# saithepaithewhyyy/Stochastic-Gradient-MCMC-for-non-linear-state-models---MTH422

Measured on AMD Instinct MI355X. Metric: SGLD steps/sec (T=1000, N=1000 particles), higher is better.
Workload: dtype f64

## Files before the change

### stochastic-gradient-mcmc-for-non-linear-state-models---mth422_amd/csrc/pfg_models.hpp

```cpp
#pragma once
#include "pfg_math.hpp"

namespace pfg {

template <int MODEL> struct ModelDims;
template <> struct ModelDims<PFG_MODEL_SVM>   { static constexpr int NS = 1, H = 3; };
template <> struct ModelDims<PFG_MODEL_GARCH> { static constexpr int NS = 2, H = 4; };
template <> struct ModelDims<PFG_MODEL_LGSSM> { static constexpr int NS = 1, H = 4; };

template <typename REAL> struct Consts {
    REAL LRinv, iLRinv, Rinv, R, logLRinv, c0;
    REAL A, C, LQinv, iLQinv, Qinv;
    REAL opt_sd, opt_prec, opt_var, opt_logvar;
    REAL mu, phi, lam, alpha, beta, gamma;
    REAL logalpha, logLQinv;
};

template <int MODEL, typename REAL>
__device__ __forceinline__ Consts<REAL> make_consts(const double *__restrict__ th) {
    Consts<double> d = {};
    d.c0 = -0.5 * LOG_2PI;
    double LRinv;
    if (MODEL == PFG_MODEL_SVM) {
        d.A = th[0]; d.LQinv = th[1]; LRinv = th[2];
    } else if (MODEL == PFG_MODEL_LGSSM) {
        d.A = th[0]; d.C = th[1]; d.LQinv = th[2]; LRinv = th[3];
    } else {
        LRinv = th[3];
        d.mu = exp(th[0]);
        d.phi = 1.0 / (1.0 + exp(-th[1]));
        d.lam = 1.0 / (1.0 + exp(-th[2]));
        d.alpha = d.mu * (1.0 - d.phi);
        d.beta = d.phi * d.lam;
        d.gamma = d.phi * (1.0 - d.lam);
    }
    d.LRinv = LRinv;
    d.iLRinv = 1.0 / LRinv;
    d.Rinv = LRinv * LRinv + 1e-16;
    d.R = 1.0 / d.Rinv;
    d.logLRinv = log(LRinv);
    if (MODEL != PFG_MODEL_GARCH) {
        d.iLQinv = 1.0 / d.LQinv;
        d.Qinv = d.LQinv * d.LQinv + 1e-16;
        d.logLQinv = log(d.LQinv);
    } else {
        d.logalpha = log(d.alpha);
    }
    if (MODEL == PFG_MODEL_LGSSM) {
        d.opt_prec = d.Qinv + (d.C * d.C) * d.Rinv;
        d.opt_sd = pow(d.opt_prec, -0.5);
        d.opt_var = 1.0 / d.Qinv + 1.0 / d.Rinv;
        d.opt_logvar = log(d.opt_var);
    }
    {
        double *f = reinterpret_cast<double *>(&d);
#pragma unroll
        for (int q = 0; q < (int)(sizeof(d) / sizeof(double)); ++q) f[q] = uniform_f64(f[q]);
    }
    Consts<REAL> c;
    c.LRinv = (REAL)d.LRinv; c.iLRinv = (REAL)d.iLRinv; c.Rinv = (REAL)d.Rinv; c.R = (REAL)d.R;
    c.logLRinv = (REAL)d.logLRinv; c.c0 = (REAL)d.c0;
    c.A = (REAL)d.A; c.C = (REAL)d.C; c.LQinv = (REAL)d.LQinv; c.iLQinv = (REAL)d.iLQinv;
    c.Qinv = (REAL)d.Qinv;
    c.opt_sd = (REAL)d.opt_sd; c.opt_prec = (REAL)d.opt_prec; c.opt_var = (REAL)d.opt_var;
    c.opt_logvar = (REAL)d.opt_logvar;
    c.mu = (REAL)d.mu; c.phi = (REAL)d.phi; c.lam = (REAL)d.lam;
    c.alpha = (REAL)d.alpha; c.beta = (REAL)d.beta; c.gamma = (REAL)d.gamma;
    c.logalpha = (REAL)d.logalpha; c.logLQinv = (REAL)d.logLQinv;
    return c;
}

template <int MODEL, int KERNEL, int STAT, typename REAL, typename MATH>
__device__ __forceinline__ void particle_step(const Consts<REAL> &c, const MATH &mth, const REAL *xp,
                                              REAL y, REAL z, REAL *xn, REAL &lw, REAL *add) {
    constexpr int H = ModelDims<MODEL>::H;
    const REAL half = (REAL)0.5;
#pragma unroll
    for (int h = 0; h < H; ++h) add[h] = (REAL)0;
    if (MODEL == PFG_MODEL_SVM) {
        REAL xpA = xp[0] * c.A;
        REAL x1 = c.iLQinv * z + xpA;
        REAL e = mth.exp_finite(-x1);
        REAL y2 = y * y;
#ifdef PFG_FAST_ALGEBRA
        const REAL k0 = c.c0 + c.logLRinv, ke = (-half * y2) * c.Rinv;
        lw = fma(ke, e, fma(-half, x1, k0));
#else
        lw = ((c.c0 + ((-half * y2) * e) * c.Rinv) + c.logLRinv) + (-half * x1);
#endif
        xn[0] = x1;
        if (STAT == PFG_STAT_SCORE) {
            REAL dx = x1 - c.A * xp[0];
            add[2] = (c.Qinv * dx) * xp[0];
            add[1] = c.iLQinv - (dx * dx) * c.LQinv;
#ifdef PFG_FAST_ALGEBRA
            add[0] = fma(-(y2 * c.LRinv), e, c.iLRinv);
#else
            REAL dy2 = y2 * e;
            add[0] = c.iLRinv - dy2 * c.LRinv;
#endif
        } else {
            add[0] = x1; add[1] = x1 * x1; add[2] = xp[0] * x1;
        }
    } else if (MODEL == PFG_MODEL_LGSSM) {
        REAL x1;
        if (KERNEL == PFG_KERNEL_PRIOR) {
            x1 = c.iLQinv * z + xp[0] * c.A;
            REAL diff = y - c.C * x1;
            lw = (c.c0 + (-half * (diff * diff)) * c.Rinv) + c.logLRinv;
        } else {
#ifdef PFG_FAST_ALGEBRA
            const REAL rprec = (REAL)1 / c.opt_prec, rvar = (REAL)1 / c.opt_var;
            REAL mp = (xp[0] * c.A) * c.Qinv + (y * c.C) * c.Rinv;
            x1 = fma(c.opt_sd, z, mp * rprec);
            REAL diff = y - c.A * xp[0];
            lw = fma(-half * (diff * diff), rvar, -half * (REAL)LOG_2PI - half * c.opt_logvar);
#else
            REAL mp = (xp[0] * c.A) * c.Qinv + (y * c.C) * c.Rinv;
            x1 = c.opt_sd * z + mp / c.opt_prec;
            REAL diff = y - c.A * xp[0];
            lw = ((-half * (diff * diff)) / c.opt_var - half * (REAL)LOG_2PI) - half * c.opt_logvar;
#endif
        }
        xn[0] = x1;
        if (STAT == PFG_STAT_SCORE) {
            REAL dx = x1 - c.A * xp[0];
            add[3] = (c.Qinv * dx) * xp[0];
            add[1] = c.iLQinv - (dx * dx) * c.LQinv;
            REAL dy = y - c.C * x1;
            add[2] = (c.Rinv * dy) * x1;
            add[0] = c.iLRinv - (dy * dy) * c.LRinv;
        } else {
            add[0] = x1; add[1] = x1 * x1; add[2] = xp[0] * x1;
        }
    } else {
        REAL xx = xp[0] * xp[0];
        REAL s2 = (c.alpha + c.beta * xx) + c.gamma * xp[1];
        REAL x1;
        if (KERNEL == PFG_KERNEL_PRIOR) {
#ifdef PFG_FAST_ALGEBRA
            x1 = mth.sqrt_pos(s2) * z;
#else
            x1 = mth.sqrt(s2) * z;
#endif
            REAL diff = y - x1;
            lw = (c.c0 + (-half * (diff * diff)) * c.Rinv) + c.logLRinv;
        } else {
#ifdef PFG_FAST_ALGEBRA
            const REAL v2 = s2 + c.R;
            const REAL rv2 = mth.rcp_pos(v2);
            const REAL var = (s2 * c.R) * rv2;
            x1 = fma(mth.sqrt_pos(var), z, var * (y * c.Rinv));
            lw = fma(-half * (y * y), rv2, c.c0) + (-half * mth.log(v2));
#else
            REAL var = (REAL)1 / (c.Rinv + (REAL)1 / s2);
            REAL mean = var * (y * c.Rinv);
            x1 = mean + mth.sqrt(var) * z;
            REAL v2 = s2 + c.R;
            lw = (c.c0 + (-half * (y * y)) / v2) + (-half * mth.log(v2));
#endif
        }
        xn[0] = x1; xn[1] = s2;
        if (STAT == PFG_STAT_SCORE) {
            REAL v = s2;
#ifdef PFG_FAST_ALGEBRA
            const REAL rv = mth.rcp_pos(v);
            const REAL gv = (-half * (v - x1 * x1)) * (rv * rv);
            const REAL omp = (REAL)1 - c.phi, oml_ = (REAL)1 - c.lam;
            add[1] = gv * (omp * c.mu);
            add[2] = (gv * fma(c.lam, xx, fma(oml_, xp[1], -c.mu))) * (omp * c.phi);
            add[3] = (gv * (xx - xp[1])) * ((c.phi * oml_) * c.lam);
            REAL dy = y - x1;
            add[0] = fma(-(dy * dy), c.LRinv, c.iLRinv);
#else
            REAL gv = (-half * (v - x1 * x1)) / (v * v);
            add[1] = (gv * ((REAL)1 - c.phi)) * c.mu;
            add[2] = ((gv * ((-c.mu + c.lam * xx) + ((REAL)1 - c.lam) * xp[1])) * ((REAL)1 - c.phi)) * c.phi;
            add[3] = (((gv * c.phi) * (xx - xp[1])) * ((REAL)1 - c.lam)) * c.lam;
            REAL dy = y - x1;
            add[0] = c.iLRinv - (dy * dy) * c.LRinv;
#endif
        } else {
            REAL x2 = x1 * x1;
            add[0] = x1; add[1] = x2; add[2] = x2 * x2;
        }
    }
}

template <int MODEL, int STAT, typename REAL>
__device__ __forceinline__ void additive_stat(const Consts<REAL> &c, const REAL *xp, const REAL *xn, REAL y,
                                              REAL aux, REAL *add) {
    constexpr int H = ModelDims<MODEL>::H;
    const REAL half = (REAL)0.5;
#pragma unroll
    for (int h = 0; h < H; ++h) add[h] = (REAL)0;
    if (STAT != PFG_STAT_SCORE) {
        if (MODEL == PFG_MODEL_GARCH) { REAL x2 = xn[0] * xn[0]; add[0] = xn[0]; add[1] = x2; add[2] = x2 * x2; }
        else { add[0] = xn[0]; add[1] = xn[0] * xn[0]; add[2] = xp[0] * xn[0]; }
        return;
    }
    if (MODEL == PFG_MODEL_SVM) {
        REAL dx = xn[0] - c.A * xp[0];
        add[2] = (c.Qinv * dx) * xp[0];
        add[1] = c.iLQinv - (dx * dx) * c.LQinv;
        add[0] = c.iLRinv - ((y * y) * aux) * c.LRinv;
    } else if (MODEL == PFG_MODEL_LGSSM) {
        REAL dx = xn[0] - c.A * xp[0];
        add[3] = (c.Qinv * dx) * xp[0];
        add[1] = c.iLQinv - (dx * dx) * c.LQinv;
        REAL dy = y - c.C * xn[0];
        add[2] = (c.Rinv * dy) * xn[0];
        add[0] = c.iLRinv - (dy * dy) * c.LRinv;
    } else {
        REAL xx = xp[0] * xp[0];
        REAL v = xn[1];
        REAL gv = (-half * (v - xn[0] * xn[0])) / (v * v);
        add[1] = (gv * ((REAL)1 - c.phi)) * c.mu;
        add[2] = ((gv * ((-c.mu + c.lam * xx) + ((REAL)1 - c.lam) * xp[1])) * ((REAL)1 - c.phi)) * c.phi;
        add[3] = (((gv * c.phi) * (xx - xp[1])) * ((REAL)1 - c.lam)) * c.lam;
        REAL dy = y - xn[0];
        add[0] = c.iLRinv - (dy * dy) * c.LRinv;
    }
}

template <int MODEL, typename REAL, typename MATH>
__device__ __forceinline__ REAL backward_log_ratio(const Consts<REAL> &c, const MATH &mth, const REAL *xp,
                                                   const REAL *xn) {
    const REAL half = (REAL)0.5;
    if (MODEL == PFG_MODEL_GARCH) {
        REAL s2 = (c.alpha + c.beta * (xp[0] * xp[0])) + c.gamma * xp[1];
        REAL ll = ((-half * (xn[0] * xn[0])) / s2 - half * (REAL)LOG_2PI) - half * mth.log(s2);
        return ll - (-half * (REAL)LOG_2PI - half * c.logalpha);
    }
    REAL diff = xn[0] - c.A * xp[0];
    REAL ll = ((-half * (diff * diff)) * c.Qinv + -half * (REAL)LOG_2PI) + c.logLQinv;
    return ll - (-half * (REAL)LOG_2PI + c.logLQinv);
}

}
```

### stochastic-gradient-mcmc-for-non-linear-state-models---mth422_amd/csrc/pfg_reg_kernel.hpp

```cpp
#pragma once
#include "pfg_models.hpp"

namespace pfg {

__host__ __device__ __forceinline__ constexpr int cdf_phys(int i) { return i + (i >> 5); }
__host__ __device__ constexpr bool fast_layout(int NT, bool PP) { return PP || NT <= 512 || NT == 1024; }

#ifndef PFG_OPT_PADSTATE
#define PFG_OPT_PADSTATE 1
#endif
template <typename REAL, int RNG> __host__ __device__ constexpr int state_pad() {
    return (PFG_OPT_PADSTATE && RNG == PFG_RNG_DEVICE) ? (int)(8 / sizeof(REAL)) : 0;
}

template <int NW> __device__ __forceinline__ void block_sync() {
    if (NW == 1) {
        __builtin_amdgcn_fence(__ATOMIC_RELEASE, "wavefront");
        __builtin_amdgcn_wave_barrier();
        __builtin_amdgcn_fence(__ATOMIC_ACQUIRE, "wavefront");
    } else {
        __syncthreads();
    }
}
template <int NT, int PPT> struct RegLayout {
    static constexpr int NW = NT / WAVE;
    static constexpr int RED = PPT * NW + NW + PFG_MAX_STAT * NW + 8;
};

template <int MODEL, typename REAL, int NT, int PPT, int RNG, bool PP, int MODE = 0>
__host__ __device__ inline size_t reg_kernel_lds_bytes(int N) {
    constexpr bool PARIS = (MODE == MODE_PARIS || MODE == MODE_N2);
    constexpr bool FAST = fast_layout(NT, PP);
    size_t NL = FAST ? (size_t)NT * PPT : (size_t)(N + WAVE - 1) / WAVE * WAVE;
    size_t NC = FAST ? (size_t)NT * PPT + (size_t)NT * PPT / 32 : NL;
    constexpr bool BLK = FAST && RNG == PFG_RNG_DEVICE && MODE == MODE_PLAIN && (PPT & (PPT - 1)) == 0;
    const size_t NLS = NL + (FAST ? state_pad<REAL, RNG>() : 0);
    return (NC * (BLK ? 4 : 8) + 15) / 16 * 16 + (PP ? 2 : 1) * NLS * (ModelDims<MODEL>::NS + ModelDims<MODEL>::H) * sizeof(REAL) +
           (size_t)RegLayout<NT, PPT>::RED * 8 + tab_bytes<REAL, RNG, FAST>() +
           (PARIS ? NL * 8 + NL * 4 + 3 * NL * 4 : 0);
}

#ifndef PFG_OCC64
#define PFG_OCC64 4
#endif
__host__ __device__ constexpr bool occ_lds4096(int NT, int PPT) { return NT * PPT == 4096 && NT < 1024; }
__host__ __device__ constexpr int occ_max(int NT, int PPT, size_t real, bool PP, bool dev4 = false) {
    if (occ_lds4096(NT, PPT)) return NT == 512 ? 2 : 1;
    if (NT == 64) return PFG_OCC64;
    return (NT >= 512 || PPT == 1 || dev4) ? 4 : ((PP && real == 8) ? 2 : 3);
}
__host__ __device__ constexpr int occ_min(int NT, int PPT, size_t real, bool PP, bool dev4 = false) {
    if (occ_lds4096(NT, PPT)) return NT == 512 ? 2 : 1;
    if (NT == 512) return 4;
    return dev4 ? 4 : ((NT == 256 && PPT == 4 && !PP) ? 3 : 1);
}
#ifndef PFG_EXP_PLAIN
#define PFG_EXP_PLAIN 0
#endif
#define PFG_TR(p) (TRACE && (p))
#ifdef PFG_FAST_ALGEBRA
#ifndef PFG_OPT_LAZYLL
#define PFG_OPT_LAZYLL 1
#endif
#ifndef PFG_OPT_RCPW
#define PFG_OPT_RCPW 1
#endif
#ifndef PFG_OPT_SEL32
#define PFG_OPT_SEL32 1
#endif
#ifndef PFG_OPT_PIVOTS
#define PFG_OPT_PIVOTS 0
#endif
#else
#undef PFG_OPT_LAZYLL
#undef PFG_OPT_RCPW
#define PFG_OPT_LAZYLL 0
#define PFG_OPT_RCPW 0
#undef PFG_OPT_SEL32
#define PFG_OPT_SEL32 0
#undef PFG_OPT_PIVOTS
#define PFG_OPT_PIVOTS 0
#endif
#ifndef PFG_OCC4
#define PFG_OCC4 1
#endif
__host__ __device__ constexpr bool occ_two(int MODEL, int NT, int PPT, size_t real, bool PP) {
    return MODEL == PFG_MODEL_GARCH && real == 8 && NT == 256 && PPT == 4 && !PP;
}
__host__ __device__ constexpr bool occ_dev4(int MODEL, int NT, int PPT, int RNG, bool PP, int MODE) {
    return PFG_OCC4 && MODEL == PFG_MODEL_SVM && NT == 256 && PPT == 4 && !PP && RNG == PFG_RNG_DEVICE && MODE == MODE_PLAIN;
}

template <int MODEL, int KERNEL, typename REAL, int NT, int PPT, int RNG, bool PP, int MODE = 0, bool TRACE = true, bool SCORE1 = false>
__global__ __launch_bounds__(NT) __attribute__((amdgpu_waves_per_eu(occ_two(MODEL, NT, PPT, sizeof(REAL), PP) ? 2 : occ_min(NT, PPT, sizeof(REAL), PP, occ_dev4(MODEL, NT, PPT, RNG, PP, MODE)), occ_two(MODEL, NT, PPT, sizeof(REAL), PP) ? 2 : occ_max(NT, PPT, sizeof(REAL), PP, occ_dev4(MODEL, NT, PPT, RNG, PP, MODE))))) void pf_reg_kernel(const pfg_dev_problem *__restrict__ probs) {
    constexpr bool PARIS = (MODE == MODE_PARIS);
    constexpr bool systematic = (MODE == MODE_SYSTEMATIC);
    constexpr bool N2 = (MODE == MODE_N2);
    static_assert(!(PARIS || N2) || PP, "PaRIS / O(N^2) need the parents intact while children are built: ping-pong buffers");
    static_assert(!systematic || RNG == PFG_RNG_DEVICE, "systematic resampling draws its offset on the device");
    constexpr int NS = ModelDims<MODEL>::NS;
    constexpr int H = ModelDims<MODEL>::H;
    constexpr int NW = NT / WAVE;
    extern __shared__ __align__(16) unsigned char smem[];

    const pfg_dev_problem &P = probs[blockIdx.x];
    const int N = P.N, T = P.T, t1 = P.t1, tL = P.tL;
    const int NL = fast_layout(NT, PP) ? NT * PPT : (N + WAVE - 1) / WAVE * WAVE;
    const int tid = threadIdx.x, lane = tid & (WAVE - 1);
    const int wave = __builtin_amdgcn_readfirstlane(tid / WAVE);
    constexpr bool ONLY_SCORE1 = PFG_EXP_PLAIN || SCORE1;
    if constexpr (SCORE1) {
        if (P.smoother != PFG_SMOOTHER_NEMETH || P.lambduh != 1.0 || P.stat != PFG_STAT_SCORE) {
            if (threadIdx.x < PFG_OUT_DOUBLES && P.out) P.out[threadIdx.x] = __builtin_nan("");
            return;
        }
    }
    const bool is_filter = !ONLY_SCORE1 && (P.smoother == PFG_SMOOTHER_FILTER);
    const int stat = ONLY_SCORE1 ? (int)PFG_STAT_SCORE : P.stat;
    const double lam_d = ONLY_SCORE1 ? 1.0 : is_filter ? 0.0 : ((P.smoother == PFG_SMOOTHER_PARIS || N2) ? 1.0 : P.lambduh);
    const REAL lam = (REAL)lam_d, oml = (REAL)(1.0 - lam_d);
    const bool needS_every = is_filter || (lam_d != 1.0);
    const gptr<const double> yv = global_ptr(P.y);
    const gptr<const double> wv = global_ptr(P.weights);
    const gptr<const double> uv = global_ptr(P.u);
    const gptr<const double> zv = global_ptr(P.z);

    constexpr bool FAST = fast_layout(NT, PP);
    constexpr bool TAB = FAST;
    constexpr bool BLK = FAST && RNG == PFG_RNG_DEVICE && MODE == MODE_PLAIN && (PPT & (PPT - 1)) == 0;
#ifndef PFG_OPT_SORTED1024
#define PFG_OPT_SORTED1024 1
#endif
    constexpr bool SORTED = PFG_OPT_SORTED1024 && BLK && NT == 1024 && PPT == 4 && !systematic && NW > 1;
#ifndef PFG_OPT_PRIO
#define PFG_OPT_PRIO 1
#endif
    constexpr int PRIO = !(PFG_OPT_PRIO && (BLK || (RNG == PFG_RNG_REPLAY && MODE == MODE_PLAIN)) && !PP && PPT == 4) ? 0 : (NT == 1024 ? 1 : (NT == 256 ? 2 : 0));
    constexpr int LOG_PPT = PPT == 1 ? 0 : (PPT == 2 ? 1 : (PPT == 4 ? 2 : (PPT == 8 ? 3 : 4)));
    static_assert(PPT <= 16, "LOG_PPT covers 1, 2, 4, 8, 16 particles per thread");
    const int NC = FAST ? NT * PPT + NT * PPT / 32 : NL;
    double *cdf = reinterpret_cast<double *>(smem);
    uint32_t *cdfu = reinterpret_cast<uint32_t *>(smem);
    REAL *buf0 = reinterpret_cast<REAL *>(smem + ((size_t)NC * (BLK ? 4 : 8) + 15) / 16 * 16);
    const int NLS = NL + (FAST ? state_pad<REAL, RNG>() : 0);
    const size_t bufsz = (size_t)(NS + H) * NLS;
    REAL *cur = buf0, *nxt = PP ? buf0 + bufsz : buf0;
#ifndef PFG_OPT_PAIRSTATE
#define PFG_OPT_PAIRSTATE 1
#endif
    constexpr bool PAIRED = PFG_OPT_PAIRSTATE && BLK && sizeof(REAL) == 8 && ((NS + H) % 2 == 0);
    auto sidx = [&](int d, int i) -> size_t {
        return PAIRED ? (size_t)(d >> 1) * (2 * (size_t)NLS) + 2 * (size_t)i + (size_t)(d & 1) : (size_t)d * NLS + (size_t)i;
    };
    double *red = reinterpret_cast<double *>(buf0 + (PP ? 2 : 1) * bufsz);
    double *red_scan = red;
    double *red_max = red + PPT * NW;
    float *red_maxf = reinterpret_cast<float *>(red_max);
    double *red_S = red_max + NW;
    double *red_W0 = red_S + PFG_MAX_STAT * NW;
    const double invN = 1.0 / (double)N;
    double *tabmem = red + RegLayout<NT, PPT>::RED;
    REAL *lwL = reinterpret_cast<REAL *>(tabmem + tab_bytes<REAL, RNG, TAB>() / 8);
    int *paris_queue = reinterpret_cast<int *>(tabmem + tab_bytes<REAL, RNG, TAB>() / 8 + NL);

    Math<REAL, TAB> mth;
    mth.t.e2 = tabmem;
    mth.t.lg = reinterpret_cast<const double2 *>(tabmem + TAB_E2);
    mth.t.sc = reinterpret_cast<const double2 *>(tabmem + TAB_E2 + 2 * TAB_LG);
    if (tab_bytes<REAL, RNG, TAB>() > 0) tab_fill(tabmem, RNG == PFG_RNG_DEVICE, tid, NT);
    if (FAST && !BLK) {
#pragma unroll
        for (int k = 0; k < PPT; ++k)
            if (k * NT + tid >= N) cdf[cdf_phys(k * NT + tid)] = 2.0;
    }
    __syncthreads();

    const Consts<REAL> c = make_consts<MODEL, REAL>(P.theta);
    int np2 = 1;
    while (np2 < N) np2 <<= 1;
    if (P.stamps && tid == 0) { P.stamps[0] = __builtin_amdgcn_s_memtime(); P.stamps[1] = __builtin_amdgcn_s_memrealtime(); }
#ifdef PFG_PHASE_STAMPS
    unsigned long long ph_acc[10] = {0, 0, 0, 0, 0, 0, 0, 0, 0, 0};
    unsigned long long ph_prev = __builtin_amdgcn_s_memtime();
#define PFG_PH(i) { const unsigned long long ph_now = __builtin_amdgcn_s_memtime(); ph_acc[i] += ph_now - ph_prev; ph_prev = ph_now; }
#define PFG_MARK(s)
#elif defined(PFG_ISA_MARKERS)
#define PFG_PH(i) asm volatile("; PFG_PHASE " #i);
#define PFG_MARK(s) asm volatile("; PFG_MARK " s);
#else
#define PFG_PH(i)
#define PFG_MARK(s)
#endif

    LaneRng rng = {};
    if (RNG == PFG_RNG_DEVICE)
        rng = lane_rng_init(P.seed, P.stream, P.step_ctr ? *P.step_ctr : 0ull, (uint32_t)tid);
    auto draw_normals = [&](REAL *zz) {
#pragma unroll
        for (int k = 0; k < PPT; k += 2) {
            REAL a, b;
            mth.normal_pair(rng.next(), rng.next(), a, b);
            zz[k] = a;
            if (k + 1 < PPT) zz[k + 1] = b;
        }
    };

    REAL lw[PPT];
    long long paris_cursor = 0;
    bool paris_overflow = false;
    constexpr bool RAWCAP = MODE == MODE_PARIS && RNG == PFG_RNG_REPLAY;
    const bool raw = RAWCAP && (P.flags & PFG_FLAG_PARIS_RAW_STREAM) != 0 && P.paris_stream != nullptr;
    bool carry_has = false;
    double *const zbuf = reinterpret_cast<double *>(paris_queue);
    long long *const raw_slots = reinterpret_cast<long long *>(red_W0 + 2);
    [[maybe_unused]] auto legacy_normals = [&]() {
        const gptr<const double> strm = global_ptr(P.paris_stream);
        const long long cap = P.paris_stream_len;
        const unsigned long long ltm = (1ull << lane) - 1ull;
        int *const wc = reinterpret_cast<int *>(red_scan);
        const int produced0 = carry_has ? 1 : 0;
        __syncthreads();
        if (carry_has && tid == 0) zbuf[0] = red_W0[1];
        const int need = (N - produced0 + 1) >> 1;
        const long long base = paris_cursor;
        int acc = 0;
        for (int round = 0; acc < need && !paris_overflow; ++round) {
            double x1[PPT], x2[PPT], r2[PPT];
            bool fl[PPT];
            int rank[PPT];
#pragma unroll
            for (int k = 0; k < PPT; ++k) {
                const long long p = base + 2 * ((long long)round * (NT * PPT) + k * NT + tid);
                const bool in = p + 1 < cap;
                const double d0 = in ? strm[p] : 0.5, d1 = in ? strm[p + 1] : 0.5;
                x1[k] = 2.0 * d0 - 1.0;
                x2[k] = 2.0 * d1 - 1.0;
                r2[k] = x1[k] * x1[k] + x2[k] * x2[k];
                fl[k] = in && !(r2[k] >= 1.0 || r2[k] == 0.0);
                const unsigned long long mk = __ballot(fl[k]);
                rank[k] = __popcll(mk & ltm);
                if (lane == 0) wc[k * NW + wave] = __popcll(mk);
            }
            __syncthreads();
            int S = 0;
#pragma unroll
            for (int k = 0; k < PPT; ++k) {
#pragma unroll
                for (int w = 0; w < NW; ++w) {
                    if (w == wave) rank[k] += S;
                    S += wc[k * NW + w];
                }
            }
#pragma unroll
            for (int k = 0; k < PPT; ++k) {
                const int q = acc + rank[k];
                if (fl[k] && q < need) {
                    const double f = sqrt(-2.0 * log(r2[k]) / r2[k]);
                    const int i0 = produced0 + 2 * q;
                    zbuf[i0] = f * x2[k];
                    const long long j = (long long)round * (NT * PPT) + k * NT + tid;
                    if (i0 + 1 < N) zbuf[i0 + 1] = f * x1[k];
                    else { red_W0[1] = f * x1[k]; raw_slots[1] = base + 2 * j; }
                    if (q == need - 1) raw_slots[0] = j;
                }
            }
            acc += S;
            if (acc < need && base + 2 * ((long long)(round + 1) * (NT * PPT)) + 1 >= cap) paris_overflow = true;
            __syncthreads();
        }
        if (need > 0 && !paris_overflow) paris_cursor = base + 2 * (raw_slots[0] + 1);
        carry_has = ((N - produced0) & 1) != 0;
    };
    if (RAWCAP && raw && (P.flags & PFG_FLAG_PARIS_RAW_CARRY)) {
        carry_has = true;
        if (tid == 0) red_W0[1] = P.paris_stream[0];
        paris_cursor = 1;
    }
    {
        double pv = P.prior_var;
        if (MODEL == PFG_MODEL_GARCH && (P.flags & PFG_FLAG_GARCH_STATIONARY_PRIOR))
            pv = (double)c.alpha / (1.0 - (double)c.beta - (double)c.gamma);
        const double sd = sqrt(pv);
        REAL z0[PPT];
        if (RNG == PFG_RNG_DEVICE) draw_normals(z0);
        if constexpr (RAWCAP) { if (raw && !P.init_x) legacy_normals(); }
#pragma unroll
        for (int k = 0; k < PPT; ++k) {
            const int i = k * NT + tid;
            lw[k] = (REAL)0;
            if (i < N) {
                REAL x[NS], s[H];
#pragma unroll
                for (int d = 0; d < NS; ++d) x[d] = (REAL)0;
#pragma unroll
                for (int h = 0; h < H; ++h) s[h] = (REAL)0;
                if (P.init_x) {
#pragma unroll
                    for (int d = 0; d < NS; ++d) x[d] = (REAL)P.init_x[(size_t)i * NS + d];
                    lw[k] = (REAL)P.init_logw[i];
                    if (P.init_stats && !is_filter) {
#pragma unroll
                        for (int h = 0; h < H; ++h) s[h] = (REAL)P.init_stats[(size_t)i * H + h];
                    }
                } else {
                    const double z = (RNG == PFG_RNG_REPLAY) ? ((RAWCAP && raw) ? zbuf[i] : P.z0[i]) : (double)z0[k];
                    x[0] = (REAL)(P.prior_mean + sd * z);
                    if (RNG == PFG_RNG_DEVICE && PFG_TR(P.trace_x) && P.rec_z0) P.rec_z0[i] = z;
                }
#pragma unroll
                for (int d = 0; d < NS; ++d) cur[sidx(d, i)] = x[d];
#pragma unroll
                for (int h = 0; h < H; ++h) cur[sidx((NS + h), i)] = s[h];
                if (PFG_TR(P.trace_x)) {
#pragma unroll
                    for (int d = 0; d < NS; ++d) P.trace_x[(size_t)i * NS + d] = (double)x[d];
                    P.trace_logw[i] = (double)lw[k];
                    if (P.trace_stats && !is_filter) {
#pragma unroll
                        for (int h = 0; h < H; ++h) P.trace_stats[(size_t)i * H + h] = (double)s[h];
                    }
                }
            }
        }
    }

    double ll = 0.0, wt_prev = 1.0, tie = 1.0;
    constexpr bool LAZYLL = PFG_OPT_LAZYLL && TAB && sizeof(REAL) == 8;
    double ll_W = 1.0, ll_w = 0.0;
    float ll_m = 0.0f;
    double filt[H], S[H];
#pragma unroll
    for (int h = 0; h < H; ++h) { filt[h] = 0.0; S[h] = 0.0; }
    double m = 0.0, W = (double)N;
    bool valid[PPT];
    int own[PPT];
#pragma unroll
    for (int k = 0; k < PPT; ++k) {
        valid[k] = (k * NT + tid) < N;
        own[k] = valid[k] ? (k * NT + tid) : (N - 1);
        if (!valid[k]) lw[k] = -INFINITY;
    }
    const int last = N - 1;

    for (int t = 0; t <= T; ++t) {
        [[maybe_unused]] double uu_raw[PPT];
        [[maybe_unused]] REAL zz_raw[PPT];
        if constexpr (RAWCAP) {
            if (raw && t < T) {
                const gptr<const double> strm = global_ptr(P.paris_stream);
                if (paris_cursor + N > P.paris_stream_len) paris_overflow = true;
#pragma unroll
                for (int k = 0; k < PPT; ++k) uu_raw[k] = paris_overflow ? 0.5 : strm[paris_cursor + own[k]];
                if (!paris_overflow) paris_cursor += N;
                legacy_normals();
#pragma unroll
                for (int k = 0; k < PPT; ++k) zz_raw[k] = (REAL)zbuf[own[k]];
            }
        }
        float ml = (float)lw[0];
#pragma unroll
        for (int k = 1; k < PPT; ++k) ml = fmaxf(ml, (float)lw[k]);
        ml = wave_max(ml);
        if (NW > 1 && lane == 0) red_maxf[wave] = ml;
        PFG_PH(0)
        block_sync<NW>();
        PFG_PH(1)
        {
            float mm = NW > 1 ? red_maxf[0] : ml;
#pragma unroll
            for (int w = 1; w < NW; ++w) mm = fmaxf(mm, red_maxf[w]);
            m = uniform_f64((double)mm);
        }
        const bool needS = needS_every || (t == T);
        double cs[PPT];
#pragma unroll
        for (int k = 0; k < PPT; ++k) cs[k] = (double)mth.exp((REAL)(lw[k] - (REAL)m));
        if (needS) {
            PFG_MARK("cold needS")
#pragma unroll
            for (int h = 0; h < H; ++h) {
                double part = 0.0;
#pragma unroll
                for (int k = 0; k < PPT; ++k) part += (double)cur[sidx((NS + h), own[k])] * cs[k];
                part = wave_sum(part);
                if (lane == 0) red_S[h * NW + wave] = part;
            }
        }
        double wave_inc = 0.0;
        float es[PPT];
        uint32_t us[PPT];
        if (BLK) {
#pragma unroll
            for (int k = 1; k < PPT; ++k) cs[k] += cs[k - 1];
            const double inc = wave_incl_scan(cs[PPT - 1]);
            const double exc = inc - cs[PPT - 1];
#pragma unroll
            for (int k = 0; k < PPT; ++k) cs[k] += exc;
            if (NW > 1 && lane == WAVE - 1) red_scan[wave] = inc;
            wave_inc = inc;
            if (SORTED && t < T) {
#pragma unroll
                for (int k = 0; k < PPT; ++k) {
                    const float e = spacing_f32(rng.next());
                    es[k] = (valid[k] ? e : 0.0f) + (k > 0 ? es[k - 1] : 0.0f);
                }
                const float eincf = wave_incl_scan_f32(es[PPT - 1]);
                const float eexc = eincf - es[PPT - 1];
#pragma unroll
                for (int k = 0; k < PPT; ++k) es[k] += eexc;
                if (lane == WAVE - 1) {
                    double einc = (double)eincf;
                    if (wave == NW - 1) einc += (double)spacing_f32(rng.next());
                    red_scan[NW + wave] = einc;
                }
            }
        } else {
#pragma unroll
            for (int k = 0; k < PPT; ++k) {
                cs[k] = wave_incl_scan(cs[k]);
                if (lane == WAVE - 1) red_scan[k * NW + wave] = cs[k];
            }
        }
        if (RNG != PFG_RNG_REPLAY && systematic && tid == 0) red_W0[0] = u01_32(rng.next());
        double uu[PPT];
        REAL zz[PPT];
        if (t < T && RNG == PFG_RNG_REPLAY) {
            if (RAWCAP && raw) {
#pragma unroll
                for (int k = 0; k < PPT; ++k) { uu[k] = uu_raw[k]; zz[k] = zz_raw[k]; }
            } else {
#pragma unroll
                for (int k = 0; k < PPT; ++k) {
                    uu[k] = uv[(size_t)t * N + own[k]];
                    zz[k] = (REAL)zv[(size_t)t * N + own[k]];
                }
            }
        }
        PFG_PH(2)
        block_sync<NW>();
        PFG_PH(3)
        if (BLK && NW == 1) {
            W = __hiloint2double(__builtin_amdgcn_readlane(__double2hiint(wave_inc), WAVE - 1),
                                 __builtin_amdgcn_readlane(__double2loint(wave_inc), WAVE - 1));
        } else if (BLK) {
            const double tot = (lane < NW) ? red_scan[lane] : 0.0;
            double inc = tot;
            inc += dpp_shr0_f64<0x111>(inc);
            inc += dpp_shr0_f64<0x112>(inc);
            if (NW > 4) { inc += dpp_shr0_f64<0x114>(inc); inc += dpp_shr0_f64<0x118>(inc); }
            const double exc = inc - tot;
            const double off = __hiloint2double(__builtin_amdgcn_readlane(__double2hiint(exc), wave),
                                                __builtin_amdgcn_readlane(__double2loint(exc), wave));
#pragma unroll
            for (int k = 0; k < PPT; ++k) cs[k] += off;
            W = __hiloint2double(__builtin_amdgcn_readlane(__double2hiint(inc), NW - 1),
                                 __builtin_amdgcn_readlane(__double2loint(inc), NW - 1));
            if (SORTED && t < T) {
                const double totE = (lane < NW) ? red_scan[NW + lane] : 0.0;
                double incE = totE;
                incE += dpp_shr0_f64<0x111>(incE);
                incE += dpp_shr0_f64<0x112>(incE);
                incE += dpp_shr0_f64<0x114>(incE);
                incE += dpp_shr0_f64<0x118>(incE);
                const double excE = incE - totE;
                const double offE = __hiloint2double(__builtin_amdgcn_readlane(__double2hiint(excE), wave),
                                                     __builtin_amdgcn_readlane(__double2loint(excE), wave));
                const double Etot = __hiloint2double(__builtin_amdgcn_readlane(__double2hiint(incE), NW - 1),
                                                     __builtin_amdgcn_readlane(__double2loint(incE), NW - 1));
                double r = __builtin_amdgcn_rcp(Etot);
                r = fma(fma(-Etot, r, 1.0), r, r);
                r = fma(fma(-Etot, r, 1.0), r, r);
                const double fe = uniform_f64(r * 4294967296.0);
#pragma unroll
                for (int k = 0; k < PPT; ++k) us[k] = cvt_u32_sat(((double)es[k] + offE) * fe);
            }
        } else if (PPT * NW <= 16) {
            double tot = (lane < PPT * NW) ? red_scan[lane] : 0.0;
            double inc = tot;
            inc += dpp_shr0_f64<0x111>(inc);
            inc += dpp_shr0_f64<0x112>(inc);
            inc += dpp_shr0_f64<0x114>(inc);
            inc += dpp_shr0_f64<0x118>(inc);
            const double exc = inc - tot;
#pragma unroll
            for (int k = 0; k < PPT; ++k) {
                const int j = k * NW + wave;
                cs[k] += __hiloint2double(__builtin_amdgcn_readlane(__double2hiint(exc), j),
                                          __builtin_amdgcn_readlane(__double2loint(exc), j));
            }
            W = __hiloint2double(__builtin_amdgcn_readlane(__double2hiint(inc), PPT * NW - 1),
                                 __builtin_amdgcn_readlane(__double2loint(inc), PPT * NW - 1));
        } else {
            double run = 0.0;
#pragma unroll
            for (int k = 0; k < PPT; ++k) {
                double off = 0.0;
#pragma unroll
                for (int w = 0; w < NW; ++w) {
                    off = (w == wave) ? run : off;
                    run += red_scan[k * NW + w];
                }
                cs[k] += off;
            }
            W = uniform_f64(run);
        }
        double invW;
        if (PFG_OPT_RCPW) {
            double r = __builtin_amdgcn_rcp(W);
            r = fma(fma(-W, r, 1.0), r, r);
            r = fma(fma(-W, r, 1.0), r, r);
            invW = uniform_f64(r);
        } else {
            invW = uniform_f64(1.0 / W);
        }
        if (needS) {
            PFG_MARK("cold needS")
#pragma unroll
            for (int h = 0; h < H; ++h) {
                double acc = 0.0;
#pragma unroll
                for (int w = 0; w < NW; ++w) acc += red_S[h * NW + w];
                S[h] = uniform_f64(acc * invW);
            }
        }
        if (wave == 0) {
            PFG_MARK("w0.25 wave0-loglik")
            const bool counts = t > 0 && (t - 1) >= t1 && (t - 1) < tL;
            if (LAZYLL) {
                const bool mine = lane == (t & (WAVE - 1));
                ll_W = mine ? W : ll_W;
                ll_w = mine ? (counts ? wt_prev : 0.0) : ll_w;
                ll_m = mine ? (float)m : ll_m;
                if ((t & (WAVE - 1)) == WAVE - 1 || t == T || PFG_TR(P.trace_ll)) {
                    PFG_MARK("cold loglik-flush")
                    const double term = ll_w * ((double)ll_m + (double)mth.log((REAL)(ll_W * invN)));
                    ll = uniform_f64(ll + wave_sum(term));
                    ll_w = 0.0;
                }
            } else if (counts) {
                ll = uniform_f64(ll + wt_prev * (m + log(W / (double)N)));
            }
            if (PFG_TR(P.trace_ll) && tid == 0) P.trace_ll[t] = ll;
        }
        if (is_filter && t > 0) {
            PFG_MARK("cold filter")
#pragma unroll
            for (int h = 0; h < H; ++h) filt[h] = uniform_f64(filt[h] + S[h]);
        }
        if (t == T) break;

        const double y_t = yv[t];
        const bool inside = (t >= t1) && (t < tL);
        const double wt = (inside && wv) ? wv[t - t1] : 1.0;
        const bool use_stat = inside && (stat != PFG_STAT_NONE);
        const bool plain = !needS_every;
        if (BLK) {
            {
                const double fixs = invW * 4294967296.0;
#pragma unroll
                for (int k = 0; k < PPT; ++k)
                    cdfu[cdf_phys(tid * PPT + k)] = cvt_u32_sat(cs[k] * fixs);
            }
        } else {
#pragma unroll
            for (int k = 0; k < PPT; ++k)
                if (valid[k]) {
                    cdf[FAST ? cdf_phys(k * NT + tid) : k * NT + tid] = cs[k] * invW;
                    if (PARIS || N2) lwL[k * NT + tid] = lw[k];
                }
        }
        PFG_PH(4)
        block_sync<NW>();
        PFG_PH(5)
        if (PRIO == 1) __builtin_amdgcn_s_setprio(2);
        if (PRIO == 2) __builtin_amdgcn_s_setprio(0);

        if (RNG != PFG_RNG_REPLAY) {
            if (systematic) {
                const double u0 = red_W0[0];
#pragma unroll
                for (int k = 0; k < PPT; ++k) uu[k] = ((double)(k * NT + tid) + u0) * invN;
            } else if (!BLK) {
#pragma unroll
                for (int k = 0; k < PPT; ++k) uu[k] = u01_32(rng.next());
            }
        }
        int anc[PPT];
#pragma unroll
        for (int k = 0; k < PPT; ++k) anc[k] = 0;
        if (BLK) {
            uint32_t ua[PPT];
#pragma unroll
            for (int k = 0; k < PPT; ++k) ua[k] = SORTED ? us[k] : rng.next();
#ifdef PFG_EXP_EVENWORDS
#pragma unroll
            for (int k = 0; k < PPT; ++k) ua[k] = (uint32_t)(((uint64_t)(tid * PPT + k) << 32) / (uint64_t)(NT * PPT)) + (ua[k] >> 12);
#endif
            if (PFG_TR(P.trace_x) && P.rec_u) {
#pragma unroll
                for (int k = 0; k < PPT; ++k)
                    if (valid[k]) P.rec_u[(size_t)t * N + k * NT + tid] = ua[k];
            }
            using lds_u32 = const __attribute__((address_space(3))) uint32_t;
            const uint32_t cdf_base = (uint32_t)(uintptr_t)(lds_u32 *)cdfu;
            uint32_t off[PPT];
#pragma unroll
            for (int k = 0; k < PPT; ++k) off[k] = cdf_base;
            constexpr bool PIVOTS = PFG_OPT_PIVOTS && NT * PPT == 1024;
            constexpr int FIRST_STEP = PIVOTS ? 128 : (NT * PPT) >> 1;
            if constexpr (PIVOTS) {
                const uint32_t p511 = __builtin_amdgcn_readfirstlane(cdfu[cdf_phys(511)]);
                const uint32_t p255 = __builtin_amdgcn_readfirstlane(cdfu[cdf_phys(255)]);
                const uint32_t p767 = __builtin_amdgcn_readfirstlane(cdfu[cdf_phys(767)]);
#pragma unroll
                for (int k = 0; k < PPT; ++k) {
                    const bool g1 = p511 <= ua[k];
                    const uint32_t t2 = g1 ? p767 : p255;
                    const bool g2 = t2 <= ua[k];
                    off[k] += (g1 ? 4u * (512 + 16) : 0u) + (g2 ? 4u * (256 + 8) : 0u);
                }
            }
#pragma unroll
            for (int step = FIRST_STEP; step >= 1; step >>= 1) {
                const int probe = step - 1 + (step >= 32 ? (step >> 5) - 1 : 0);
                const int adv = step + (step >> 5);
                uint32_t cv[PPT];
#pragma unroll
                for (int k = 0; k < PPT; ++k) cv[k] = *(lds_u32 *)(uintptr_t)(off[k] + 4u * probe);
                if constexpr (PFG_OPT_SEL32 && NT >= 512) {
                uint32_t cand[PPT];
#pragma unroll
                for (int k = 0; k < PPT; ++k) cand[k] = off[k] + 4u * adv;
#pragma unroll
                for (int k = 0; k < PPT; ++k)
                    asm("v_cmp_le_u32_e32 vcc, %1, %2\n\tv_cndmask_b32_e32 %0, %3, %4, vcc"
                        : "=v"(off[k]) : "v"(cv[k]), "v"(ua[k]), "v"(off[k]), "v"(cand[k]) : "vcc");
                } else {
#pragma unroll
                for (int k = 0; k < PPT; ++k) off[k] += (cv[k] <= ua[k]) ? 4u * adv : 0u;
                }
            }
#pragma unroll
            for (int k = 0; k < PPT; ++k) {
                uint32_t p = (off[k] - cdf_base) >> 2;
                p -= __umul24(p, 993u) >> 15;
                anc[k] = (int)(((p << (NT == 256 ? 8 : (NT == 512 ? 9 : (NT == 1024 ? 10 : 6)))) & (uint32_t)((PPT - 1) * NT)) | (p >> LOG_PPT));
            }
        } else if (FAST) {
            using lds_f64 = const __attribute__((address_space(3))) double;
            const uint32_t cdf_base = (uint32_t)(uintptr_t)(lds_f64 *)cdf;
            uint32_t off[PPT];
#pragma unroll
            for (int k = 0; k < PPT; ++k) off[k] = cdf_base;
#pragma unroll
            for (int step = (NT * PPT) >> 1; step >= 1; step >>= 1) {
                const int probe = step - 1 + (step >= 32 ? (step >> 5) - 1 : 0);
                const int adv = step + (step >> 5);
                double cv[PPT];
#pragma unroll
                for (int k = 0; k < PPT; ++k) cv[k] = *(lds_f64 *)(uintptr_t)(off[k] + 8u * probe);
#pragma unroll
                for (int k = 0; k < PPT; ++k) off[k] += (cv[k] <= uu[k]) ? 8u * adv : 0u;
            }
#pragma unroll
            for (int k = 0; k < PPT; ++k) {
                const uint32_t p = (off[k] - cdf_base) >> 3;
                anc[k] = (int)(p - (__umul24(p, 993u) >> 15));
            }
        } else {
            for (int step = np2 >> 1; step >= 1; step >>= 1) {
#pragma unroll
                for (int k = 0; k < PPT; ++k) {
                    int idx = anc[k] + step - 1;
                    idx = idx < last ? idx : last;
                    anc[k] += (cdf[idx] <= uu[k]) ? step : 0;
                }
            }
        }
#pragma unroll
        for (int k = 0; k < PPT; ++k) anc[k] = anc[k] < last ? anc[k] : last;
#ifdef PFG_EXP_OWNGATHER
#pragma unroll
        for (int k = 0; k < PPT; ++k) { asm volatile("" :: "v"(anc[k])); anc[k] = valid[k] ? k * NT + tid : 0; }
#endif
        if (RNG == PFG_RNG_REPLAY) {
#pragma unroll
            for (int k = 0; k < PPT; ++k) {
                const double hi = cdf[FAST ? cdf_phys(anc[k]) : anc[k]] - uu[k];
                const double lo = anc[k] > 0 ? uu[k] - cdf[FAST ? cdf_phys(anc[k] - 1) : anc[k] - 1] : 1.0;
                const double mg = hi < lo ? hi : lo;
                tie = (valid[k] && mg < tie) ? mg : tie;
            }
        }
        PFG_PH(6)
        auto slots = [&](auto stat_tag) {
            constexpr int STAT = decltype(stat_tag)::value;
            if (STAT != PFG_STAT_SCORE) { PFG_MARK("cold sufficient-statistics") }
            REAL xp[PPT][NS], sp[PPT][H];
#pragma unroll
            for (int k = 0; k < PPT; ++k) {
                if constexpr (PAIRED) {
                    typedef double dv2 __attribute__((ext_vector_type(2)));
                    REAL rec[NS + H];
#pragma unroll
                    for (int p = 0; p < (NS + H) / 2; ++p) {
                        const dv2 v = *reinterpret_cast<const dv2 *>(&cur[sidx(2 * p, anc[k])]);
                        rec[2 * p] = (REAL)v.x; rec[2 * p + 1] = (REAL)v.y;
                    }
#pragma unroll
                    for (int d = 0; d < NS; ++d) xp[k][d] = rec[d];
#pragma unroll
                    for (int h = 0; h < H; ++h) sp[k][h] = rec[NS + h];
                } else {
#pragma unroll
                for (int d = 0; d < NS; ++d) xp[k][d] = cur[sidx(d, anc[k])];
#pragma unroll
                for (int h = 0; h < H; ++h) sp[k][h] = cur[sidx((NS + h), anc[k])];
                }
            }
            PFG_PH(7)
            if (PRIO == 1) __builtin_amdgcn_s_setprio(0);
            if (PRIO == 2) __builtin_amdgcn_s_setprio(2);
            if (!PP) block_sync<NW>();
            PFG_PH(8)
            if (RNG != PFG_RNG_REPLAY) {
                draw_normals(zz);
                if (PFG_TR(P.trace_x) && P.rec_z) {
#pragma unroll
                    for (int k = 0; k < PPT; ++k)
                        if (valid[k]) P.rec_z[(size_t)t * N + k * NT + tid] = (double)zz[k];
                }
            }
            auto children = [&](auto upd_tag) {
                constexpr int UPD = decltype(upd_tag)::value;
                if (UPD == 1) { PFG_MARK("cold children-outside-window") }
                if (UPD == 2) { PFG_MARK("cold children-general") }
#pragma unroll
                for (int k = 0; k < PPT; ++k) {
                    REAL xn[NS], add[H], lwn;
                    particle_step<MODEL, KERNEL, STAT, REAL>(c, mth, xp[k], (REAL)y_t, zz[k], xn, lwn, add);
                    lw[k] = valid[k] ? lwn : (REAL)(-INFINITY);
                    if (UPD == 0) {
#pragma unroll
                        for (int h = 0; h < H; ++h) sp[k][h] = sp[k][h] + add[h] * (REAL)wt;
                    } else if (UPD == 2) {
#pragma unroll
                        for (int h = 0; h < H; ++h) {
                            const REAL a = use_stat ? add[h] * (REAL)wt : (REAL)0;
                            const REAL sm = (lam * sp[k][h] + oml * (REAL)S[h]) + a;
                            sp[k][h] = is_filter ? a : sm;
                        }
                    }
                    if ((FAST && NT < 1024) || valid[k]) {
                        const int i = k * NT + tid;
                        if constexpr (PAIRED) {
                            typedef double dv2 __attribute__((ext_vector_type(2)));
                            REAL rec[NS + H];
#pragma unroll
                            for (int d = 0; d < NS; ++d) rec[d] = xn[d];
#pragma unroll
                            for (int h = 0; h < H; ++h) rec[NS + h] = sp[k][h];
#pragma unroll
                            for (int p = 0; p < (NS + H) / 2; ++p) {
                                dv2 v;
                                v.x = (double)rec[2 * p]; v.y = (double)rec[2 * p + 1];
                                *reinterpret_cast<dv2 *>(&nxt[sidx(2 * p, i)]) = v;
                            }
                        } else {
#pragma unroll
                        for (int d = 0; d < NS; ++d) nxt[sidx(d, i)] = xn[d];
#pragma unroll
                        for (int h = 0; h < H; ++h) nxt[sidx((NS + h), i)] = sp[k][h];
                        }
                    }
                }
            };
            if (!plain) children(std::integral_constant<int, 2>{});
            else if (use_stat) children(std::integral_constant<int, 0>{});
            else children(std::integral_constant<int, 1>{});
        };
        auto paris_slots = [&](auto stat_tag) {
            constexpr int STAT = decltype(stat_tag)::value;
            const int Nt = P.Ntilde, R = P.max_accept_reject;
            const double *__restrict__ const pidx = P.paris_idx_u;
            const double *__restrict__ const pacc = P.paris_acc_u;
            const double *__restrict__ const pman = P.paris_man_u;
            int *queue = paris_queue;
            int *qcount = reinterpret_cast<int *>(red_max) + NW;
            if (RNG != PFG_RNG_REPLAY) draw_normals(zz);
            REAL xn[PPT][NS], lwn[PPT], aux[PPT], sacc[PPT][H];
#pragma unroll
            for (int k = 0; k < PPT; ++k) {
                REAL xp[NS], add[H];
#pragma unroll
                for (int d = 0; d < NS; ++d) xp[d] = cur[sidx(d, anc[k])];
                particle_step<MODEL, KERNEL, STAT, REAL>(c, mth, xp, (REAL)y_t, zz[k], xn[k], lwn[k], add);
                aux[k] = (MODEL == PFG_MODEL_SVM) ? mth.exp(-xn[k][0]) : (REAL)0;
#pragma unroll
                for (int h = 0; h < H; ++h) sacc[k][h] = (REAL)0;
                if (valid[k]) {
#pragma unroll
                    for (int d = 0; d < NS; ++d) nxt[sidx(d, k * NT + tid)] = xn[k][d];
                }
            }
            int *const wq0 = paris_queue + NL + wave * (PPT * WAVE);
            int *const wq1 = paris_queue + 2 * NL + wave * (PPT * WAVE);
            int *const Jres = paris_queue + 3 * NL;
            const unsigned long long ltmask = (1ull << lane) - 1ull;
            const bool ordered = RNG == PFG_RNG_REPLAY && P.paris_stream != nullptr;
            for (int j = 0; j < Nt; ++j) {
                int *qa = wq0, *qb = wq1;
                int cnt = 0;
                if (!ordered) {
#pragma unroll
                for (int k = 0; k < PPT; ++k) {
                    const unsigned long long mk = __ballot(valid[k]);
                    if (valid[k]) qa[cnt + __popcll(mk & ltmask)] = k * NT + tid;
                    cnt += __popcll(mk);
                }
                }
                auto candidate = [&](int child, int round, bool act, int &Iout) {
                    double u1, u2;
                    if (RNG == PFG_RNG_REPLAY) {
                        const size_t at = (((size_t)t * Nt + j) * R + (act ? round : 0)) * N + child;
                        u1 = pidx[at]; u2 = pacc[at];
                    } else { u1 = u01_32(rng.next()); u2 = u01_32(rng.next()); }
                    int I = 0;
#pragma unroll
                    for (int step = (NT * PPT) >> 1; step >= 1; step >>= 1) {
                        const int probe = step - 1 + (step >= 32 ? (step >> 5) - 1 : 0);
                        I += (cdf[I + probe] <= u1) ? step + (step >> 5) : 0;
                    }
                    I -= (I * 993) >> 15;
                    I = I < last ? I : last;
                    REAL xI[NS], xc[NS];
#pragma unroll
                    for (int d = 0; d < NS; ++d) { xI[d] = cur[sidx(d, I)]; xc[d] = nxt[sidx(d, child)]; }
                    const double thr = (double)mth.exp(backward_log_ratio<MODEL, REAL>(c, mth, xI, xc));
                    Iout = I;
                    return act && u2 <= thr;
                };
                int r0 = 0;
                while (cnt > 0 && r0 < R) {
                    __builtin_amdgcn_wave_barrier();
                    int ncnt = 0;
                    if (cnt > WAVE / 2) {
                        for (int e0 = 0; e0 < cnt; e0 += WAVE) {
                            const int e = e0 + lane;
                            const bool act = e < cnt;
                            const int child = qa[act ? e : 0];
                            int I;
                            const bool acc = candidate(child, r0, act, I);
                            if (acc) Jres[child] = I;
                            const bool rej = act && !acc;
                            const unsigned long long mk = __ballot(rej);
                            if (rej) qb[ncnt + __popcll(mk & ltmask)] = child;
                            ncnt += __popcll(mk);
                        }
                        r0 += 1;
// ... 389 lines not shown
```

Before: 288,900.

## Use stale max-shift for SVM weights and compute gather byte addresses directly

For the SVM prior kernel at NT=256, PPT=4, the per-step block-wide max reduction and its barrier are removed. The weights are instead shifted by the max computed in the previous step. If the new max drifts more than 512 from the stale one, a cold path recomputes the weights, statistics and scan. Separately, ancestor indices from the CDF search are converted straight into LDS byte offsets for the paired-state gather, which saves index arithmetic. The stale shift relies on bounded drift between steps and adds a retry path that costs extra work whenever it fires.

```diff
diff --git a/stochastic-gradient-mcmc-for-non-linear-state-models---mth422_amd/csrc/pfg_models.hpp b/stochastic-gradient-mcmc-for-non-linear-state-models---mth422_amd/csrc/pfg_models.hpp
--- a/stochastic-gradient-mcmc-for-non-linear-state-models---mth422_amd/csrc/pfg_models.hpp
+++ b/stochastic-gradient-mcmc-for-non-linear-state-models---mth422_amd/csrc/pfg_models.hpp
@@ -70,6 +70,17 @@
     return c;
 }
 
+template <typename REAL>
+__device__ __forceinline__ REAL svm_logw(const Consts<REAL> &c, REAL x1, REAL e, REAL y2) {
+    const REAL half = (REAL)0.5;
+#ifdef PFG_FAST_ALGEBRA
+    const REAL k0 = c.c0 + c.logLRinv, ke = (-half * y2) * c.Rinv;
+    return fma(ke, e, fma(-half, x1, k0));
+#else
+    return ((c.c0 + ((-half * y2) * e) * c.Rinv) + c.logLRinv) + (-half * x1);
+#endif
+}
+
 template <int MODEL, int KERNEL, int STAT, typename REAL, typename MATH>
 __device__ __forceinline__ void particle_step(const Consts<REAL> &c, const MATH &mth, const REAL *xp,
                                               REAL y, REAL z, REAL *xn, REAL &lw, REAL *add) {
@@ -82,12 +93,7 @@
         REAL x1 = c.iLQinv * z + xpA;
         REAL e = mth.exp_finite(-x1);
         REAL y2 = y * y;
-#ifdef PFG_FAST_ALGEBRA
-        const REAL k0 = c.c0 + c.logLRinv, ke = (-half * y2) * c.Rinv;
-        lw = fma(ke, e, fma(-half, x1, k0));
-#else
-        lw = ((c.c0 + ((-half * y2) * e) * c.Rinv) + c.logLRinv) + (-half * x1);
-#endif
+        lw = svm_logw(c, x1, e, y2);
         xn[0] = x1;
         if (STAT == PFG_STAT_SCORE) {
             REAL dx = x1 - c.A * xp[0];
diff --git a/stochastic-gradient-mcmc-for-non-linear-state-models---mth422_amd/csrc/pfg_reg_kernel.hpp b/stochastic-gradient-mcmc-for-non-linear-state-models---mth422_amd/csrc/pfg_reg_kernel.hpp
--- a/stochastic-gradient-mcmc-for-non-linear-state-models---mth422_amd/csrc/pfg_reg_kernel.hpp
+++ b/stochastic-gradient-mcmc-for-non-linear-state-models---mth422_amd/csrc/pfg_reg_kernel.hpp
@@ -54,6 +54,12 @@
     if (NT == 512) return 4;
     return dev4 ? 4 : ((NT == 256 && PPT == 4 && !PP) ? 3 : 1);
 }
+#ifndef PFG_OPT_STALESHIFT
+#define PFG_OPT_STALESHIFT 1
+#endif
+#ifndef PFG_OPT_GATHERADDR
+#define PFG_OPT_GATHERADDR 1
+#endif
 #ifndef PFG_EXP_PLAIN
 #define PFG_EXP_PLAIN 0
 #endif
@@ -149,6 +155,14 @@
 #define PFG_OPT_PAIRSTATE 1
 #endif
     constexpr bool PAIRED = PFG_OPT_PAIRSTATE && BLK && sizeof(REAL) == 8 && ((NS + H) % 2 == 0);
+    constexpr bool STALE = PFG_OPT_STALESHIFT && BLK && MODEL == PFG_MODEL_SVM && KERNEL == PFG_KERNEL_PRIOR && NT == 256 && PPT == 4 &&
+                           !PP && sizeof(REAL) == 8;
+#ifdef PFG_EXP_OWNGATHER
+    constexpr bool GADDR = false;
+#else
+    constexpr bool GADDR = PFG_OPT_GATHERADDR && BLK && PAIRED && NT == 256 && PPT == 4 && MODEL == PFG_MODEL_SVM && !PP;
+#endif
+    static_assert(!GADDR || 4 * (NT * PPT + NT * PPT / 32) * 993 < (1 << 23), "GADDR: rel * 993 must fit the 24-bit multiply");
     auto sidx = [&](int d, int i) -> size_t {
         return PAIRED ? (size_t)(d >> 1) * (2 * (size_t)NLS) + 2 * (size_t)i + (size_t)(d & 1) : (size_t)d * NLS + (size_t)i;
     };
@@ -341,6 +355,20 @@
         if (!valid[k]) lw[k] = -INFINITY;
     }
     const int last = N - 1;
+    [[maybe_unused]] float m_next = 0.0f;
+    if constexpr (STALE) {
+        float ml = (float)lw[0];
+#pragma unroll
+        for (int k = 1; k < PPT; ++k) ml = fmaxf(ml, (float)lw[k]);
+        ml = wave_max(ml);
+        if (lane == 0) red_maxf[wave] = ml;
+        block_sync<NW>();
+        float mm = red_maxf[0];
+#pragma unroll
+        for (int w = 1; w < NW; ++w) mm = fmaxf(mm, red_maxf[w]);
+        m = uniform_f64((double)mm);
+        block_sync<NW>();
+    }
 
     for (int t = 0; t <= T; ++t) {
         [[maybe_unused]] double uu_raw[PPT];
@@ -363,9 +391,9 @@
         ml = wave_max(ml);
         if (NW > 1 && lane == 0) red_maxf[wave] = ml;
         PFG_PH(0)
-        block_sync<NW>();
+        if constexpr (!STALE) block_sync<NW>();
         PFG_PH(1)
-        {
+        if constexpr (!STALE) {
             float mm = NW > 1 ? red_maxf[0] : ml;
 #pragma unroll
             for (int w = 1; w < NW; ++w) mm = fmaxf(mm, red_maxf[w]);
@@ -455,6 +483,53 @@
             for (int k = 0; k < PPT; ++k) cs[k] += off;
             W = __hiloint2double(__builtin_amdgcn_readlane(__double2hiint(inc), NW - 1),
                                  __builtin_amdgcn_readlane(__double2loint(inc), NW - 1));
+            if constexpr (STALE) {
+                float mm = red_maxf[0];
+#pragma unroll
+                for (int w = 1; w < NW; ++w) mm = fmaxf(mm, red_maxf[w]);
+                m_next = __builtin_bit_cast(float, __builtin_amdgcn_readfirstlane(__builtin_bit_cast(int, mm)));
+                if (t > 0 && !(fabsf(m_next - (float)m) <= 512.0f)) {
+                    PFG_MARK("cold stale-shift-retry")
+                    block_sync<NW>();
+                    m = uniform_f64((double)m_next);
+                    const REAL y_p = (REAL)yv[t - 1], y2_p = y_p * y_p;
+#pragma unroll
+                    for (int k = 0; k < PPT; ++k) {
+                        const REAL x1 = cur[sidx(0, own[k])];
+                        const REAL lwk = valid[k] ? svm_logw(c, x1, mth.exp_finite(-x1), y2_p) : (REAL)(-INFINITY);
+                        cs[k] = (double)mth.exp((REAL)(lwk - (REAL)m));
+                    }
+                    if (needS) {
+#pragma unroll
+                        for (int h = 0; h < H; ++h) {
+                            double part = 0.0;
+#pragma unroll
+                            for (int k = 0; k < PPT; ++k) part += (double)cur[sidx((NS + h), own[k])] * cs[k];
+                            part = wave_sum(part);
+                            if (lane == 0) red_S[h * NW + wave] = part;
+                        }
+                    }
+#pragma unroll
+                    for (int k = 1; k < PPT; ++k) cs[k] += cs[k - 1];
+                    const double inc2 = wave_incl_scan(cs[PPT - 1]);
+                    const double exc2 = inc2 - cs[PPT - 1];
+#pragma unroll
+                    for (int k = 0; k < PPT; ++k) cs[k] += exc2;
+                    if (lane == WAVE - 1) red_scan[wave] = inc2;
+                    block_sync<NW>();
+                    const double tot2 = (lane < NW) ? red_scan[lane] : 0.0;
+                    double incw = tot2;
+                    incw += dpp_shr0_f64<0x111>(incw);
+                    incw += dpp_shr0_f64<0x112>(incw);
+                    const double excw = incw - tot2;
+                    const double off2 = __hiloint2double(__builtin_amdgcn_readlane(__double2hiint(excw), wave),
+                                                         __builtin_amdgcn_readlane(__double2loint(excw), wave));
+#pragma unroll
+                    for (int k = 0; k < PPT; ++k) cs[k] += off2;
+                    W = __hiloint2double(__builtin_amdgcn_readlane(__double2hiint(incw), NW - 1),
+                                         __builtin_amdgcn_readlane(__double2loint(incw), NW - 1));
+                }
+            }
             if (SORTED && t < T) {
                 const double totE = (lane < NW) ? red_scan[NW + lane] : 0.0;
                 double incE = totE;
@@ -548,6 +623,7 @@
             for (int h = 0; h < H; ++h) filt[h] = uniform_f64(filt[h] + S[h]);
         }
         if (t == T) break;
+        if constexpr (STALE) m = uniform_f64((double)m_next);
 
         const double y_t = yv[t];
         const bool inside = (t >= t1) && (t < tL);
@@ -586,8 +662,9 @@
             }
         }
         int anc[PPT];
-#pragma unroll
-        for (int k = 0; k < PPT; ++k) anc[k] = 0;
+        [[maybe_unused]] uint32_t gaddr[PPT];
+#pragma unroll
+        for (int k = 0; k < PPT; ++k) { anc[k] = 0; gaddr[k] = 0u; }
         if (BLK) {
             uint32_t ua[PPT];
 #pragma unroll
@@ -640,6 +717,18 @@
                 for (int k = 0; k < PPT; ++k) off[k] += (cv[k] <= ua[k]) ? 4u * adv : 0u;
                 }
             }
+            if constexpr (GADDR) {
+#pragma unroll
+                for (int k = 0; k < PPT; ++k) {
+                    const uint32_t rel = off[k] - cdf_base;
+                    const uint32_t q = __umul24(rel, 993u) >> 17;
+                    uint32_t p4;
+                    asm("v_mad_i32_i24 %0, %1, -4, %2" : "=v"(p4) : "v"(q), "v"(rel));
+                    const uint32_t a = __umul24(p4, 1025u) & 0x3ff0u;
+                    gaddr[k] = min(a, 16u * (uint32_t)last);
+                    if constexpr (TRACE) anc[k] = (int)(gaddr[k] >> 4);
+                }
+            } else
 #pragma unroll
             for (int k = 0; k < PPT; ++k) {
                 uint32_t p = (off[k] - cdf_base) >> 2;
@@ -704,7 +793,13 @@
                     REAL rec[NS + H];
 #pragma unroll
                     for (int p = 0; p < (NS + H) / 2; ++p) {
-                        const dv2 v = *reinterpret_cast<const dv2 *>(&cur[sidx(2 * p, anc[k])]);
+                        dv2 v;
+                        if constexpr (GADDR) {
+                            using lds_byte = const __attribute__((address_space(3))) unsigned char;
+                            v = *(const __attribute__((address_space(3))) dv2 *)((lds_byte *)cur + gaddr[k] + (uint32_t)(p * 16 * NLS));
+                        } else {
+                            v = *reinterpret_cast<const dv2 *>(&cur[sidx(2 * p, anc[k])]);
+                        }
                         rec[2 * p] = (REAL)v.x; rec[2 * p + 1] = (REAL)v.y;
                     }
 #pragma unroll
```

Measured after the change: 294,900, median of 6. +2.1%, better.
